# zhangmozhe/Deep-Exemplar-based-Video-Colorization

Hardware: AMD Instinct MI355X
Metric: colorized frames/sec/GPU at 216x384; correlation HBM GB/s vs roofline (higher is better)
Workload: dtype f32

## Files before the change

deep-exemplar-based-video-colorization_amd/csrc/norm_pool.hip:

```cpp
#include "common.h"
#include <algorithm>

thread_local char g_dvc_err[512] = {0};
char* dvc_err_buf() { return g_dvc_err; }

extern "C" int dvc_abi_version(void) { return DVC_ABI_VERSION; }
extern "C" const char* dvc_last_error(void) { return g_dvc_err; }

__device__ __forceinline__ double wave_sum_d(double v) {
#pragma unroll
    for (int off = 32; off > 0; off >>= 1) v += __shfl_xor(v, off, 64);
    return v;
}
__device__ __forceinline__ float wave_sum_f(float v) {
#pragma unroll
    for (int off = 32; off > 0; off >>= 1) v += __shfl_xor(v, off, 64);
    return v;
}

__device__ __forceinline__ double block_sum_d(double v, double* red) {
    v = wave_sum_d(v);
    int lane = threadIdx.x & 63, wave = threadIdx.x >> 6;
    __syncthreads();
    if (lane == 0) red[wave] = v;
    __syncthreads();
    double t = 0.0;
    int nw = blockDim.x >> 6;
    for (int i = 0; i < nw; ++i) t += red[i];
    return t;
}

__device__ __forceinline__ void plane_stats(const float* __restrict__ xp, int HW, float eps, float cs,
                                            double* red , float* sc_out, float* sh_out) {
    constexpr int VT = 1024;
    const int tid = threadIdx.x, nt = blockDim.x;
    const int nv = VT / nt;
    double s[4] = {0.0, 0.0, 0.0, 0.0}, q[4] = {0.0, 0.0, 0.0, 0.0};
    const int HW4 = ((reinterpret_cast<uintptr_t>(xp) & 15) == 0) ? (HW & ~3) : 0;
#pragma unroll
    for (int k = 0; k < 4; ++k) {
        if (k < nv) {
            const int v = tid + k * nt;
            int i = v * 4;
            for (; i + 3 * VT * 4 < HW4; i += 4 * VT * 4) {
                float4 x8[4];
#pragma unroll
                for (int u = 0; u < 4; ++u) x8[u] = *reinterpret_cast<const float4*>(xp + i + u * (VT * 4));
#pragma unroll
                for (int u = 0; u < 4; ++u) {
                    double a = x8[u].x, b = x8[u].y, cc = x8[u].z, d = x8[u].w;
                    s[k] += (a + b) + (cc + d);
                    q[k] += (a * a + b * b) + (cc * cc + d * d);
                }
            }
            for (; i < HW4; i += VT * 4) {
                float4 x4 = *reinterpret_cast<const float4*>(xp + i);
                double a = x4.x, b = x4.y, cc = x4.z, d = x4.w;
                s[k] += (a + b) + (cc + d);
                q[k] += (a * a + b * b) + (cc * cc + d * d);
            }
            for (int i = HW4 + v; i < HW; i += VT) {
                double a = xp[i];
                s[k] += a;
                q[k] += a * a;
            }
        }
    }
    const int lane = tid & 63, wave = tid >> 6, nw = nt >> 6;
#pragma unroll
    for (int k = 0; k < 4; ++k) {
        if (k < nv) {
            const double sk = wave_sum_d(s[k]), qk = wave_sum_d(q[k]);
            if (lane == 0) {
                red[wave + k * nw] = sk;
                red[16 + wave + k * nw] = qk;
            }
        }
    }
    __syncthreads();
    if (tid == 0) {
        double S = 0.0, Q = 0.0;
        for (int i = 0; i < VT / 64; ++i) {
            S += red[i];
            Q += red[16 + i];
        }
        const double mean = S / (double)HW;
        double var = Q / (double)HW - mean * mean;
        var = var < 0.0 ? 0.0 : var;
        const double rstd = 1.0 / sqrt(var + (double)eps);
        const double sc = rstd * (double)cs;
        red[32] = sc;
        red[33] = -mean * sc;
        red[34] = mean;
        red[35] = rstd;
    }
    __syncthreads();
    *sc_out = (float)red[32];
    *sh_out = (float)red[33];
}

__global__ __launch_bounds__(1024) void instnorm_stats_kernel(const float* __restrict__ x, int C, int HW,
                                                              long x_bs, float eps,
                                                              const float* __restrict__ chan_scale,
                                                              float* __restrict__ scale,
                                                              float* __restrict__ shift) {
    __shared__ double red[36];
    const int p = blockIdx.x;
    const int n = p / C, c = p - n * C;
    float sc, sh;
    plane_stats(x + (long)n * x_bs + (long)c * HW, HW, eps, chan_scale ? chan_scale[c] : 1.f, red, &sc, &sh);
    if (threadIdx.x == 0) {
        scale[p] = sc;
        shift[p] = sh;
    }
}

static int instnorm_block(int HW) { return HW >= 32768 ? 1024 : HW >= 8192 ? 512 : 256; }

extern "C" int dvc_instnorm_stats(const float* x, int32_t N, int32_t C, int32_t HW,
                                  int64_t x_batch_stride, float eps, const float* chan_scale,
                                  float* scale, float* shift, dvcStream stream) {
    DVC_REQUIRE(x && scale && shift && N > 0 && C > 0 && HW > 0, "dvc_instnorm_stats: bad argument");
    long bs = x_batch_stride ? x_batch_stride : (long)C * HW;
    hipLaunchKernelGGL(instnorm_stats_kernel, dim3(N * C), dim3(instnorm_block(HW)), 0, (hipStream_t)stream,
                       x, C, HW, bs, eps, chan_scale, scale, shift);
    DVC_CHECK_LAUNCH("dvc_instnorm_stats");
    return 0;
}

__device__ __forceinline__ void instnorm_apply_plane(const float* xp, const int p, const int n, const int c, double* red,
                                                     const float* __restrict__ res, const float* __restrict__ slope_ptr,
                                                     const float* __restrict__ chan_scale, float eps, int C, int H, int W,
                                                     int up, int sub, int rpad, long res_bs, long y_bs, float* __restrict__ y,
                                                     float* __restrict__ scale, float* __restrict__ shift,
                                                     const float* __restrict__ chan_scale2, int sub2, long y2_bs,
                                                     float* __restrict__ y2) {
    float sc, sh;
    plane_stats(xp, H * W, eps, chan_scale ? chan_scale[c] : 1.f, red, &sc, &sh);
    if (threadIdx.x == 0 && scale) {
        scale[p] = sc;
        shift[p] = sh;
    }
    if (y2) {
        const double sc2d = red[35] * (chan_scale2 ? (double)chan_scale2[c] : 1.0);
        const float sc2 = (float)sc2d, sh2 = (float)(-red[34] * sc2d);
        const int OH2 = sub2 == 2 ? (H + 1) / 2 : H, OW2 = sub2 == 2 ? (W + 1) / 2 : W;
        float* y2p = y2 + (long)n * y2_bs + (long)c * OH2 * OW2;
        for (int i = threadIdx.x; i < OH2 * OW2; i += blockDim.x) {
            const int oy = i / OW2, ox = i - oy * OW2;
            y2p[i] = xp[(oy * sub2) * W + ox * sub2] * sc2 + sh2;
        }
    }
    const bool has_act = slope_ptr != nullptr;
    const float slope = has_act ? *slope_ptr : 1.f;
    const float* rp = res ? res + (long)n * res_bs + (long)c * H * W : nullptr;
    const int VH = sub == 2 ? (H + 1) / 2 : H * up, VW = sub == 2 ? (W + 1) / 2 : W * up;
    const int OH = VH + 2 * rpad, OW = VW;
    float* yp = y + (long)n * y_bs + (long)c * OH * OW;
    const int total = OH * OW, nt = blockDim.x;
    if (up == 1 && sub == 1 && rpad == 0) {
        const bool v4 = ((reinterpret_cast<uintptr_t>(xp) | reinterpret_cast<uintptr_t>(yp) |
                          reinterpret_cast<uintptr_t>(rp)) & 15) == 0;
        const int T4 = v4 ? (total & ~3) : 0;
        auto piece = [&](const float4& v, const float4& r, int i) {
            float o[4] = {v.x * sc + sh, v.y * sc + sh, v.z * sc + sh, v.w * sc + sh};
            if (rp) { o[0] += r.x; o[1] += r.y; o[2] += r.z; o[3] += r.w; }
            if (has_act) {
#pragma unroll
                for (int k = 0; k < 4; ++k) o[k] = o[k] >= 0.f ? o[k] : o[k] * slope;
            }
            *reinterpret_cast<float4*>(yp + i) = make_float4(o[0], o[1], o[2], o[3]);
        };
        int i = threadIdx.x * 4;
        for (; i + nt * 4 < T4; i += 2 * nt * 4) {
            float4 v[2], r[2];
#pragma unroll
            for (int u = 0; u < 2; ++u) {
                v[u] = *reinterpret_cast<const float4*>(xp + i + u * nt * 4);
                r[u] = rp ? *reinterpret_cast<const float4*>(rp + i + u * nt * 4) : make_float4(0.f, 0.f, 0.f, 0.f);
            }
#pragma unroll
            for (int u = 0; u < 2; ++u) piece(v[u], r[u], i + u * nt * 4);
        }
        for (; i < T4; i += nt * 4) {
            const float4 v = *reinterpret_cast<const float4*>(xp + i);
            const float4 r = rp ? *reinterpret_cast<const float4*>(rp + i) : make_float4(0.f, 0.f, 0.f, 0.f);
            piece(v, r, i);
        }
        for (int i = T4 + threadIdx.x; i < total; i += nt) {
            float v = xp[i] * sc + sh;
            if (rp) v += rp[i];
            if (has_act) v = v >= 0.f ? v : v * slope;
            yp[i] = v;
        }
        return;
    }
    for (int i = threadIdx.x; i < total; i += nt) {
        int oy = i / OW, ox = i - oy * OW;
        int uy = oy - rpad;
        uy = uy < 0 ? 0 : (uy >= VH ? VH - 1 : uy);
        int sy = sub == 2 ? uy * 2 : (up == 1 ? uy : uy / up);
        int sx = sub == 2 ? ox * 2 : (up == 1 ? ox : ox / up);
        float v = xp[sy * W + sx] * sc + sh;
        if (rp) v += rp[sy * W + sx];
        if (has_act) v = v >= 0.f ? v : v * slope;
        yp[i] = v;
    }
}


__global__ __launch_bounds__(1024) void instnorm_apply_kernel(const float* __restrict__ x,
                                                              const float* __restrict__ res,
                                                              const float* __restrict__ slope_ptr,
                                                              const float* __restrict__ chan_scale, float eps,
                                                              int C, int H, int W, int up, int sub, int rpad,
                                                              long x_bs, long res_bs, long y_bs,
                                                              float* __restrict__ y, float* __restrict__ scale,
                                                              float* __restrict__ shift,
                                                              const float* __restrict__ chan_scale2, int sub2,
                                                              long y2_bs, float* __restrict__ y2) {
    __shared__ double red[36];
    const int p = blockIdx.x;
    const int n = p / C, c = p - n * C;
    instnorm_apply_plane(x + (long)n * x_bs + (long)c * H * W, p, n, c, red, res, slope_ptr, chan_scale, eps, C, H, W, up, sub,
                         rpad, res_bs, y_bs, y, scale, shift, chan_scale2, sub2, y2_bs, y2);
}

__global__ __launch_bounds__(1024) void instnorm_apply_partials_kernel(const float* __restrict__ part, int S, long slab,
                                                                       const float* __restrict__ bias, int act, float act_slope,
                                                                       const float* __restrict__ act_slope_ptr,
                                                                       const float* __restrict__ res,
                                                                       const float* __restrict__ slope_ptr,
                                                                       const float* __restrict__ chan_scale, float eps,
                                                                       int C, int H, int W, int up, int sub, int rpad,
                                                                       long res_bs, long y_bs,
                                                                       float* __restrict__ y, float* __restrict__ scale,
                                                                       float* __restrict__ shift,
                                                                       const float* __restrict__ chan_scale2, int sub2,
                                                                       long y2_bs, float* __restrict__ y2) {
    __shared__ double red[36];
// ... 28 lines not shown
    }
    __syncthreads();
    instnorm_apply_plane(plane, p, n, c, red, res, slope_ptr, chan_scale, eps, C, H, W, up, sub, rpad, res_bs, y_bs, y, scale,
                         shift, chan_scale2, sub2, y2_bs, y2);
}

extern "C" int dvc_instnorm_apply(const float* x, const float* residual, const float* slope_ptr,
                                  const float* chan_scale, float eps, int32_t N, int32_t C, int32_t H,
                                  int32_t W, int32_t up, int32_t sub, int32_t rpad, int64_t x_batch_stride,
                                  int64_t res_batch_stride, int64_t y_batch_stride, float* y,
                                  float* scale_out, float* shift_out, const float* chan_scale2, int32_t sub2,
                                  float* y2, dvcStream stream) {
    DVC_REQUIRE(x && y && N > 0 && C > 0 && H > 0 && W > 0, "dvc_instnorm_apply: bad argument");
    DVC_REQUIRE(!y2 || ((sub2 == 1 || sub2 == 2) && y2 != x && y2 != y), "dvc_instnorm_apply: bad second output");
    DVC_REQUIRE(!(y2 && x == y), "dvc_instnorm_apply: a second output excludes in-place operation");
    DVC_REQUIRE(up >= 1 && up <= 4 && (sub == 1 || sub == 2) && rpad >= 0 && !(up != 1 && sub != 1),
                "dvc_instnorm_apply: bad up/sub/rpad");
    DVC_REQUIRE(!(residual && (up != 1 || sub != 1)), "dvc_instnorm_apply: residual requires up == sub == 1");
    DVC_REQUIRE((scale_out == nullptr) == (shift_out == nullptr), "dvc_instnorm_apply: scale/shift come together");
    DVC_REQUIRE(!(x == y && (up != 1 || sub != 1 || rpad != 0)), "dvc_instnorm_apply: in place needs up == sub == 1, rpad == 0");
    const long VH = sub == 2 ? (H + 1) / 2 : (long)H * up, VW = sub == 2 ? (W + 1) / 2 : (long)W * up;
    const long OH = VH + 2 * rpad, OW = VW;
    long xbs = x_batch_stride ? x_batch_stride : (long)C * H * W;
    long rbs = res_batch_stride ? res_batch_stride : (long)C * H * W;
    long ybs = y_batch_stride ? y_batch_stride : (long)C * OH * OW;
    hipLaunchKernelGGL(instnorm_apply_kernel, dim3(N * C), dim3(instnorm_block(H * W)), 0, (hipStream_t)stream,
                       x, residual, slope_ptr, chan_scale, eps, C, H, W, up, sub, rpad, xbs, rbs, ybs, y,
                       scale_out, shift_out, chan_scale2, y2 ? sub2 : 1,
                       (long)C * (sub2 == 2 ? (H + 1) / 2 : H) * (sub2 == 2 ? (W + 1) / 2 : W), y2);
    DVC_CHECK_LAUNCH("dvc_instnorm_apply");
    return 0;
}

extern "C" int dvc_instnorm_apply_partials(const float* part, int32_t S, const float* bias, int32_t act, float act_slope,
                                           const float* act_slope_ptr, const float* residual, const float* slope_ptr,
                                           const float* chan_scale, float eps, int32_t N, int32_t C, int32_t H, int32_t W,
                                           int32_t up, int32_t sub, int32_t rpad, int64_t res_batch_stride,
                                           int64_t y_batch_stride, float* y, float* scale_out, float* shift_out,
                                           const float* chan_scale2, int32_t sub2, float* y2, dvcStream stream) {
    DVC_REQUIRE(part && y && S >= 1 && S <= 8 && N > 0 && C > 0 && H > 0 && W > 0, "dvc_instnorm_apply_partials: bad argument");
    DVC_REQUIRE((long)H * W <= 16384, "dvc_instnorm_apply_partials: plane of %d x %d does not fit the LDS image (<= 16384 elements)", H, W);
    DVC_REQUIRE(act == DVC_ACT_NONE || act == DVC_ACT_RELU || act == DVC_ACT_PRELU || act == DVC_ACT_LEAKY,
                "dvc_instnorm_apply_partials: unsupported activation %d", act);
    DVC_REQUIRE(!y2 || ((sub2 == 1 || sub2 == 2) && y2 != y), "dvc_instnorm_apply_partials: bad second output");
    DVC_REQUIRE(up >= 1 && up <= 4 && (sub == 1 || sub == 2) && rpad >= 0 && !(up != 1 && sub != 1),
                "dvc_instnorm_apply_partials: bad up/sub/rpad");
    DVC_REQUIRE(!(residual && (up != 1 || sub != 1)), "dvc_instnorm_apply_partials: residual requires up == sub == 1");
    DVC_REQUIRE((scale_out == nullptr) == (shift_out == nullptr), "dvc_instnorm_apply_partials: scale/shift come together");
    const long VH = sub == 2 ? (H + 1) / 2 : (long)H * up, VW = sub == 2 ? (W + 1) / 2 : (long)W * up;
    const long OH = VH + 2 * rpad, OW = VW;
    const long rbs = res_batch_stride ? res_batch_stride : (long)C * H * W;
    const long ybs = y_batch_stride ? y_batch_stride : (long)C * OH * OW;
    hipLaunchKernelGGL(instnorm_apply_partials_kernel, dim3(N * C), dim3(H * W >= 4096 ? 1024 : 512), (size_t)H * W * sizeof(float),
                       (hipStream_t)stream, part, S, (long)N * C * H * W, bias, act, act_slope, act_slope_ptr, residual, slope_ptr,
                       chan_scale, eps, C, H, W, up, sub, rpad, rbs, ybs, y, scale_out, shift_out, chan_scale2, y2 ? sub2 : 1,
                       (long)C * (sub2 == 2 ? (H + 1) / 2 : H) * (sub2 == 2 ? (W + 1) / 2 : W), y2);
    DVC_CHECK_LAUNCH("dvc_instnorm_apply_partials");
    return 0;
}

#define INSTNORM_GROUP_MAX 4
struct InstNormGroupArgs {
    DvcInstNormItem item[INSTNORM_GROUP_MAX];
    int start[INSTNORM_GROUP_MAX + 1];
    int n;
};
// ... 372 lines not shown
```

deep-exemplar-based-video-colorization_amd/dvc_amd/_lib.py:

```python
import ctypes
import os

_HERE = os.path.dirname(os.path.abspath(__file__))
DEBUG_BUILD = os.environ.get("DVC_DEBUG_LIB", "0") == "1"
LIB_PATH = os.path.join(_HERE, "libdvc_hip_debug.so" if DEBUG_BUILD else "libdvc_hip.so")
ABI_VERSION = 20

c_float_p = ctypes.c_void_p
c_i32 = ctypes.c_int32
c_i64 = ctypes.c_int64


class DvcConvDesc(ctypes.Structure):
    _fields_ = [
        ("N", c_i32), ("Cin", c_i32), ("H", c_i32), ("W", c_i32),
        ("Cout", c_i32), ("ksize", c_i32), ("stride", c_i32), ("dil", c_i32),
        ("pad", c_i32), ("pad_mode", c_i32), ("in_up", c_i32), ("in_sub", c_i32),
        ("act", c_i32), ("act_slope", ctypes.c_float), ("in_prelu", c_i32), ("cfg", c_i32), ("split_k", c_i32),
        ("x_batch_stride", c_i64), ("y_batch_stride", c_i64), ("res_batch_stride", c_i64),
        ("flags", c_i32), ("w_batch_stride", c_i64),
    ]


class DvcConvGroupItem(ctypes.Structure):
# ... 12 lines not shown
        ("N", c_i32), ("C", c_i32), ("H", c_i32), ("W", c_i32), ("up", c_i32), ("sub", c_i32), ("rpad", c_i32),
        ("x_batch_stride", c_i64), ("res_batch_stride", c_i64), ("y_batch_stride", c_i64), ("y", ctypes.c_void_p),
    ]


_VP = ctypes.c_void_p
SIGNATURES = {
    "dvc_abi_version": (ctypes.c_int, []),
    "dvc_last_error": (ctypes.c_char_p, []),
    "dvc_conv2d_out_hw": (ctypes.c_int, [ctypes.POINTER(DvcConvDesc), ctypes.POINTER(c_i32), ctypes.POINTER(c_i32)]),
    "dvc_conv2d": (ctypes.c_int, [ctypes.POINTER(DvcConvDesc), _VP, _VP, _VP, _VP, _VP, _VP, _VP, _VP, _VP, _VP,
                                  ctypes.c_size_t, _VP]),
    "dvc_winograd_weight_floats": (ctypes.c_size_t, [c_i32, c_i32]),
    "dvc_winograd_pack_weight": (ctypes.c_int, [_VP, c_i32, c_i32, _VP, _VP]),
    "dvc_conv2d_winograd_split": (ctypes.c_int, [ctypes.POINTER(DvcConvDesc), ctypes.c_size_t, ctypes.POINTER(c_i32),
                                                ctypes.POINTER(c_i32)]),
    "dvc_conv2d_winograd": (ctypes.c_int, [ctypes.POINTER(DvcConvDesc), _VP, _VP, _VP, _VP, _VP, _VP, _VP,
                                           ctypes.c_size_t, _VP]),
    "dvc_conv2d_winograd_pool": (ctypes.c_int, [ctypes.POINTER(DvcConvDesc), _VP, _VP, _VP, _VP, _VP, _VP, c_i64, _VP,
                                                ctypes.c_size_t, _VP]),
    "dvc_conv2d_winograd_dual": (ctypes.c_int, [ctypes.POINTER(DvcConvDesc), ctypes.POINTER(DvcConvDesc), _VP, _VP, _VP, _VP, _VP,
                                                _VP, _VP, ctypes.c_size_t, _VP]),
    "dvc_conv2d_ws_eligible": (ctypes.c_int, [ctypes.POINTER(DvcConvDesc)]),
    "dvc_conv2d_ws_pack_weight": (ctypes.c_int, [_VP, c_i32, c_i32, _VP, _VP]),
    "dvc_conv2d_ws": (ctypes.c_int, [ctypes.POINTER(DvcConvDesc), _VP, _VP, _VP, _VP, _VP, _VP]),
    "dvc_conv2d_winograd_group": (ctypes.c_int, [ctypes.POINTER(DvcConvGroupItem), c_i32, _VP]),
    "dvc_instnorm_apply_group": (ctypes.c_int, [ctypes.POINTER(DvcInstNormItem), c_i32, _VP]),
    "dvc_conv1x1_small": (ctypes.c_int, [_VP, _VP, _VP, c_i32, c_i32, c_i32, c_i32, c_i32, _VP, _VP]),
    "dvc_instnorm_stats": (ctypes.c_int, [_VP, c_i32, c_i32, c_i32, c_i64, ctypes.c_float, _VP, _VP, _VP, _VP]),
    "dvc_affine_act": (ctypes.c_int, [_VP, _VP, _VP, _VP, _VP, c_i32, c_i32, c_i32, c_i32, c_i32, c_i32,
                                      c_i64, c_i64, c_i64, _VP, _VP]),
    "dvc_instnorm_apply": (ctypes.c_int, [_VP, _VP, _VP, _VP, ctypes.c_float, c_i32, c_i32, c_i32, c_i32, c_i32,
                                          c_i32, c_i32, c_i64, c_i64, c_i64, _VP, _VP, _VP, _VP, c_i32, _VP, _VP]),
    "dvc_cx_prepare": (ctypes.c_int, [_VP, _VP, c_i32, c_i32, c_i32, c_i32, ctypes.c_float, _VP, _VP, _VP, _VP]),
    "dvc_cx_rows": (ctypes.c_int, [_VP, c_i32, c_i64, c_i64, c_i32, c_i32, ctypes.c_float, _VP, _VP, _VP, _VP, _VP, _VP]),
    "dvc_cx_colmax": (ctypes.c_int, [_VP, c_i32, c_i64, c_i64, _VP, _VP, c_i32, c_i32, c_i32, ctypes.c_float, _VP, _VP, _VP]),
    "dvc_cx_finish": (ctypes.c_int, [_VP, c_i32, c_i32, _VP, _VP, _VP]),
    "dvc_cx_rows_tq": (ctypes.c_int, [_VP, c_i32, c_i64, c_i64, c_i64, _VP, _VP, _VP, c_i32, c_i32, c_i32, ctypes.c_float, _VP, _VP,
                                      _VP]),
    "dvc_cx_ds": (ctypes.c_int, [_VP, c_i32, c_i64, c_i64, c_i64, _VP, _VP, _VP, _VP, _VP, _VP, _VP, _VP, _VP, ctypes.c_float, c_i32,
                                 c_i32, c_i32, c_i32, c_i32, ctypes.c_float, _VP, _VP, _VP]),
    "dvc_cx_normalize_bwd": (ctypes.c_int, [_VP, _VP, _VP, c_i32, c_i32, c_i32, ctypes.c_float, _VP, _VP]),
    "dvc_instnorm_apply_partials": (ctypes.c_int, [_VP, c_i32, _VP, c_i32, ctypes.c_float, _VP, _VP, _VP, _VP, ctypes.c_float,
                                                   c_i32, c_i32, c_i32, c_i32, c_i32, c_i32, c_i32, c_i64, c_i64, _VP, _VP, _VP,
                                                   _VP, c_i32, _VP, _VP]),
    "dvc_maxpool2x2": (ctypes.c_int, [_VP, c_i32, c_i32, c_i32, _VP, _VP]),
    "dvc_avgpool2x2": (ctypes.c_int, [_VP, c_i32, c_i32, c_i32, _VP, _VP]),
    "dvc_avgpool4x4": (ctypes.c_int, [_VP, c_i32, c_i32, c_i32, _VP, _VP]),
    "dvc_upsample_nearest": (ctypes.c_int, [_VP, c_i32, c_i32, c_i32, c_i32, _VP, _VP]),
    "dvc_channel_l2norm": (ctypes.c_int, [_VP, c_i32, c_i32, c_i32, ctypes.c_float, _VP, _VP]),
    "dvc_channel_l2norm_multi": (ctypes.c_int, [_VP, _VP, _VP, _VP, c_i32, c_i32, ctypes.c_float, _VP]),
    "dvc_gray2rgb": (ctypes.c_int, [_VP, c_i32, c_i32, c_i64, _VP, _VP]),
    "dvc_lab2rgb": (ctypes.c_int, [_VP, c_i32, c_i32, ctypes.c_float, _VP, _VP]),
    "dvc_pack_color_input": (ctypes.c_int, [_VP, c_i64, _VP, _VP, _VP, c_i64, _VP, c_i64, c_i32, c_i32, _VP, _VP]),
    "dvc_upsample_bilinear2x": (ctypes.c_int, [_VP, c_i32, c_i32, c_i32, ctypes.c_float, _VP, _VP]),
    "dvc_lum_guide_u8": (ctypes.c_int, [_VP, c_i64, _VP, _VP]),
    "dvc_fgs_workspace_bytes": (ctypes.c_size_t, [c_i32, c_i32, c_i32, c_i32, c_i32]),
    "dvc_fgs_filter": (ctypes.c_int, [_VP, _VP, c_i32, c_i32, c_i32, c_i32, ctypes.c_float, ctypes.c_float, c_i32,
                                      ctypes.c_float, _VP, _VP, ctypes.c_size_t, _VP]),
    "dvc_lab2rgb_u8": (ctypes.c_int, [_VP, _VP, c_i32, c_i32, _VP, _VP]),
    "dvc_rgb8_to_lab": (ctypes.c_int, [_VP, c_i32, c_i32, _VP, _VP]),
    "dvc_center_pad_workspace_bytes": (ctypes.c_size_t, [c_i32, c_i32]),
    "dvc_center_pad_is_fused": (ctypes.c_int, [c_i32, c_i32, c_i32, c_i32]),
    "dvc_center_pad": (ctypes.c_int, [_VP, c_i32, c_i32, c_i32, c_i32, _VP, _VP, ctypes.c_size_t, _VP]),
    "dvc_corr_prepare": (ctypes.c_int, [_VP, c_i32, c_i32, c_i32, ctypes.c_float, _VP, _VP, _VP]),
    "dvc_corr_workspace_bytes": (ctypes.c_size_t, [c_i32, c_i32]),
# ... 86 lines not shown
```

deep-exemplar-based-video-colorization_amd/dvc_amd/ops.py:

```python
import ctypes
import os as _os
import sys
from typing import NamedTuple

import torch

from . import _lib
from ._lib import DvcConvDesc, DvcConvGroupItem, DvcInstNormItem

ACT_NONE, ACT_RELU, ACT_PRELU, ACT_LEAKY, ACT_TANH128 = 0, 1, 2, 3, 4
PAD_ZERO, PAD_REFLECT = 0, 1
EPS64 = sys.float_info.epsilon


def _p(t):
    return None if t is None else ctypes.c_void_p(t.data_ptr())


def _pv(t):
    return None if t is None else t.data_ptr()


_raw_stream = getattr(torch._C, "_cuda_getCurrentRawStream", None)
_raw_device = getattr(torch._C, "_cuda_getDevice", None)
# ... 107 lines not shown
    _Switch("fold_merge", "set_fold_merge", "_fold_merge", "DVC_FOLD_MERGE", "1", _on_if_1, True),
    _Switch("batch_plan_enabled", None, "_batch_plan", None, "0", _on_if_1, True),
    _Switch("direct_layers", None, "DEFAULT_DIRECT_LAYERS", "DVC_DIRECT_LAYERS", None, _layer_names, True),
)


def _flag_functions(var, getter, setter):
    g = globals()

    def get():
        return g[var]

    def set_(flag=True):
        g[var] = bool(flag)
    get.__name__ = get.__qualname__ = getter
    set_.__name__ = set_.__qualname__ = setter
    return get, set_


for _sw in _SWITCHES:
    globals()[_sw.var] = _sw.parse(_os.environ.get(_sw.env, _sw.default) if _sw.env else _sw.default)
    if _sw.setter:
        globals()[_sw.getter], globals()[_sw.setter] = _flag_functions(_sw.var, _sw.getter, _sw.setter)
del _sw


def launch_epoch():
    g = globals()
    return tuple(g[sw.getter]() for sw in _SWITCHES if sw.launch)


def autotune_enabled():
    return _autotune


def set_autotune(flag=True):
    global _autotune
    _autotune = bool(flag)
    if _autotune:
        _load_tuned()


def conv_algo():
    return _conv_algo


def set_conv_algo(algo):
    global _conv_algo
    if algo not in ("auto", "speed", "direct", "winograd"):
        raise ValueError("conv algo must be 'auto', 'speed', 'direct' or 'winograd'")
    _conv_algo = algo


def exemplar_memo_enabled():
    return _exemplar_memo != "off"


def exemplar_memo_mode():
    return _exemplar_memo


def set_exemplar_memo(flag=True):
    global _exemplar_memo
    _exemplar_memo = "verify" if flag == "verify" else ("on" if flag else "off")


# ... 504 lines not shown
    _need_all(x=x, chan_scale=chan_scale)
    N, C, H, W = x.shape
    scale = torch.empty(N * C, device=x.device, dtype=torch.float32)
    shift = torch.empty(N * C, device=x.device, dtype=torch.float32)
    _lib.check(lib.dvc_instnorm_stats(_p(x), N, C, H * W, 0, float(eps), _p(chan_scale), _p(scale), _p(shift),
                                      _stream()), "dvc_instnorm_stats")
    return scale, shift


def affine_act(x, scale, shift, *, residual=None, slope_t=None, up=1, rpad=0, out=None, out_batch_stride=0):
    lib = _lib.load()
    _need_all(x=x, scale=scale, shift=shift, residual=residual, slope=slope_t)
    N, C, H, W = x.shape
    if out is None:
        out = torch.empty((N, C, H * up + 2 * rpad, W * up), device=x.device, dtype=torch.float32)
    _lib.check(lib.dvc_affine_act(_p(x), _p(scale), _p(shift), _p(residual), _p(slope_t), N, C, H, W, up, rpad,
                                  0, 0, out_batch_stride, _p(out), _stream()), "dvc_affine_act")
    return out


def _instnorm_prep(x, chan_scale, residual, slope_t, up, sub, rpad, out):
    part = x if isinstance(x, ConvPartials) else None
    if part is not None:
        part.check_live()
    _need_all(x=None if part is not None else x, chan_scale=chan_scale, residual=residual, slope=slope_t)
    N, C, H, W = part.shape if part is not None else x.shape
    dev = part.device if part is not None else x.device
    VH, VW = ((H + 1) // 2, (W + 1) // 2) if sub == 2 else (H * up, W * up)
    if out is None:
        out = torch.empty((N, C, VH + 2 * rpad, VW), device=dev, dtype=torch.float32)
    return part, N, C, H, W, dev, out


def instnorm_apply(x, *, eps=1e-5, chan_scale=None, residual=None, slope_t=None, up=1, sub=1, rpad=0, out=None,
                   out_batch_stride=0, second=None, scale_out=None):
    lib = _lib.load()
    assert not isinstance(out, ConvPartials)
    part, N, C, H, W, dev, out = _instnorm_prep(x, chan_scale, residual, slope_t, up, sub, rpad, out)
    cs2, sub2, y2 = None, 1, None
    if second is not None:
        cs2, sub2 = second
        _need(cs2, "chan_scale2")
        y2 = torch.empty((N, C, (H + 1) // 2, (W + 1) // 2) if sub2 == 2 else (N, C, H, W), device=dev,
                         dtype=torch.float32)
    if part is not None:
        assert scale_out is None, "scale_out: materialise the convolution's output first (defer_reduce=False)"
        _lib.check(lib.dvc_instnorm_apply_partials(ctypes.c_void_p(part.data_ptr()), part.S, _p(part.bias), part.act,
                                                   part.act_slope, _p(part.act_slope_t), _p(residual), _p(slope_t),
                                                   _p(chan_scale), float(eps), N, C, H, W, up, sub, rpad, 0, out_batch_stride,
                                                   _p(out), None, None, _p(cs2), sub2, _p(y2), _stream()),
                   "dvc_instnorm_apply_partials")
        return out if second is None else (out, y2)
    shift_out = None
    if scale_out is not None:
        _need(scale_out, "scale_out")
        assert scale_out.numel() == N * C, (scale_out.shape, N, C)
        shift_out = torch.empty_like(scale_out)
    _lib.check(lib.dvc_instnorm_apply(_p(x), _p(residual), _p(slope_t), _p(chan_scale), float(eps), N, C, H, W, up,
                                      sub, rpad, 0, 0, out_batch_stride, _p(out), _p(scale_out), _p(shift_out), _p(cs2), sub2,
                                      _p(y2), _stream()),
               "dvc_instnorm_apply")
    return out if second is None else (out, y2)


def instnorm_apply_group(items):
    n = len(items)
    if not (_group_heads and 2 <= n <= 4):
        return [instnorm_apply(it["x"], **{k: v for k, v in it.items() if k != "x"}) for it in items]
    lib = _lib.load()
    arr = (DvcInstNormItem * n)()
    outs = []
    for i, it in enumerate(items):
        x = it["x"]
        residual, slope_t, chan_scale = it.get("residual"), it.get("slope_t"), it.get("chan_scale")
        up, sub, rpad = it.get("up", 1), it.get("sub", 1), it.get("rpad", 0)
        part, N, C, H, W, _dev, out = _instnorm_prep(x, chan_scale, residual, slope_t, up, sub, rpad, it.get("out"))
        a = arr[i]
        a.x = part.data_ptr() if part is not None else x.data_ptr()
        a.S = part.S if part is not None else 0
        a.bias = _pv(part.bias) if part is not None else None
        a.act = part.act if part is not None else ACT_NONE
        a.act_slope = part.act_slope if part is not None else 0.0
        a.act_slope_ptr = _pv(part.act_slope_t) if part is not None else None
        a.residual, a.slope_ptr, a.chan_scale = _pv(residual), _pv(slope_t), _pv(chan_scale)
        a.eps = float(it.get("eps", 1e-5))
        a.N, a.C, a.H, a.W, a.up, a.sub, a.rpad = N, C, H, W, up, sub, rpad
        a.x_batch_stride, a.res_batch_stride, a.y_batch_stride = 0, 0, it.get("out_batch_stride", 0)
        a.y = out.data_ptr()
        outs.append(out)
    _lib.check(lib.dvc_instnorm_apply_group(arr, n, _stream()), "dvc_instnorm_apply_group")
    return outs


def _pool(fn_name, x, k):
    lib = _lib.load()
    _need(x, "x")
    N, C, H, W = x.shape
    y = torch.empty((N, C, H // k, W // k), device=x.device, dtype=torch.float32)
    _lib.check(getattr(lib, fn_name)(_p(x), N * C, H, W, _p(y), _stream()), fn_name)
    return y

# ... 475 lines not shown
```

include/dvc_hip.h:

```cpp
#ifndef DVC_HIP_H
#define DVC_HIP_H

#include <stddef.h>
#include <stdint.h>

#ifdef __cplusplus
extern "C" {
#endif

#pragma GCC visibility push(default)

typedef void* dvcStream;

#define DVC_ABI_VERSION 20

int dvc_abi_version(void);
const char* dvc_last_error(void);

enum { DVC_ACT_NONE = 0, DVC_ACT_RELU = 1, DVC_ACT_PRELU = 2, DVC_ACT_LEAKY = 3, DVC_ACT_TANH128 = 4 };
enum { DVC_PAD_ZERO = 0, DVC_PAD_REFLECT = 1 };

typedef struct DvcConvDesc {
    int32_t N, Cin, H, W;
    int32_t Cout;
// ... 52 lines not shown

typedef struct DvcConvGroupItem {
    DvcConvDesc d;
    const float* x;
    const float* u_packed;
    const float* bias;
    const float* act_slope_ptr;
    const float* residual;
    float* y;
    void* workspace;
    size_t workspace_bytes;
} DvcConvGroupItem;
int dvc_conv2d_winograd_group(const DvcConvGroupItem* items, int32_t n_items, dvcStream stream);

int dvc_conv1x1_small(const float* x, const float* w, const float* bias, int32_t N, int32_t Cin,
                      int32_t HW, int32_t Cout, int32_t act, float* y, dvcStream stream);

int dvc_instnorm_stats(const float* x, int32_t N, int32_t C, int32_t HW, int64_t x_batch_stride,
                       float eps, const float* chan_scale, float* scale, float* shift,
                       dvcStream stream);

int dvc_affine_act(const float* x, const float* scale, const float* shift, const float* residual,
                   const float* slope_ptr, int32_t N, int32_t C, int32_t H, int32_t W, int32_t up,
                   int32_t rpad, int64_t x_batch_stride, int64_t res_batch_stride,
                   int64_t y_batch_stride, float* y, dvcStream stream);

int dvc_instnorm_apply(const float* x, const float* residual , const float* slope_ptr ,
                       const float* chan_scale , float eps, int32_t N, int32_t C, int32_t H,
                       int32_t W, int32_t up, int32_t sub, int32_t rpad, int64_t x_batch_stride,
                       int64_t res_batch_stride, int64_t y_batch_stride, float* y,
                       float* scale_out, float* shift_out,
                       const float* chan_scale2 , int32_t sub2, float* y2 ,
                       dvcStream stream);
int dvc_instnorm_apply_partials(const float* part, int32_t S, const float* bias, int32_t act, float act_slope,
                                const float* act_slope_ptr, const float* residual, const float* slope_ptr,
                                const float* chan_scale, float eps, int32_t N, int32_t C, int32_t H, int32_t W, int32_t up,
                                int32_t sub, int32_t rpad, int64_t res_batch_stride, int64_t y_batch_stride, float* y,
                                float* scale_out, float* shift_out, const float* chan_scale2, int32_t sub2, float* y2,
                                dvcStream stream);

typedef struct DvcInstNormItem {
    const float* x;
    int32_t S;
    const float* bias;
    int32_t act;
    float act_slope;
    const float* act_slope_ptr;
    const float* residual;
    const float* slope_ptr;
    const float* chan_scale;
    float eps;
    int32_t N, C, H, W, up, sub, rpad;
    int64_t x_batch_stride, res_batch_stride, y_batch_stride;
    float* y;
} DvcInstNormItem;
int dvc_instnorm_apply_group(const DvcInstNormItem* items, int32_t n_items, dvcStream stream);

int dvc_maxpool2x2(const float* x, int32_t planes, int32_t H, int32_t W, float* y, dvcStream stream);
int dvc_avgpool2x2(const float* x, int32_t planes, int32_t H, int32_t W, float* y, dvcStream stream);
int dvc_avgpool4x4(const float* x, int32_t planes, int32_t H, int32_t W, float* y, dvcStream stream);
int dvc_upsample_nearest(const float* x, int32_t planes, int32_t H, int32_t W, int32_t f, float* y,
                         dvcStream stream);
int dvc_channel_l2norm(const float* x, int32_t N, int32_t C, int32_t HW, float eps, float* y,
                       dvcStream stream);
#define DVC_L2NORM_MAX_TENSORS 8
int dvc_channel_l2norm_multi(const float* const* x, float* const* y, const int32_t* C, const int32_t* HW,
// ... 121 lines not shown
```

Baseline: 432.1.

## Split instance norm across workgroups for large planes with few channels

Adds a two-kernel instance-norm path. A stats kernel spreads each plane's sum and sum-of-squares over up to 16 workgroups into a workspace, then an apply kernel reduces them and normalizes slabs of the plane across many workgroups. It is chosen automatically when there are few planes of large spatial size, to fill the GPU instead of using one block per plane. It costs an extra launch and a second read of the input.

Measured after the change: 432.5 (median of 2 runs). No clear change (+0.1%).

```diff
diff --git a/deep-exemplar-based-video-colorization_amd/csrc/norm_pool.hip b/deep-exemplar-based-video-colorization_amd/csrc/norm_pool.hip
--- a/deep-exemplar-based-video-colorization_amd/csrc/norm_pool.hip
+++ b/deep-exemplar-based-video-colorization_amd/csrc/norm_pool.hip
@@ -30,42 +30,62 @@
     return t;
 }
 
+__device__ __forceinline__ void vthread_sums(const float* __restrict__ xp, int HW, int HW4, int v, double& s, double& q) {
+    constexpr int VT = 1024;
+    int i = v * 4;
+    for (; i + 3 * VT * 4 < HW4; i += 4 * VT * 4) {
+        float4 x8[4];
+#pragma unroll
+        for (int u = 0; u < 4; ++u) x8[u] = *reinterpret_cast<const float4*>(xp + i + u * (VT * 4));
+#pragma unroll
+        for (int u = 0; u < 4; ++u) {
+            double a = x8[u].x, b = x8[u].y, cc = x8[u].z, d = x8[u].w;
+            s += (a + b) + (cc + d);
+            q += (a * a + b * b) + (cc * cc + d * d);
+        }
+    }
+    for (; i < HW4; i += VT * 4) {
+        float4 x4 = *reinterpret_cast<const float4*>(xp + i);
+        double a = x4.x, b = x4.y, cc = x4.z, d = x4.w;
+        s += (a + b) + (cc + d);
+        q += (a * a + b * b) + (cc * cc + d * d);
+    }
+    for (int i = HW4 + v; i < HW; i += VT) {
+        double a = xp[i];
+        s += a;
+        q += a * a;
+    }
+}
+__device__ __forceinline__ int plane_hw4(const float* xp, int HW) {
+    return ((reinterpret_cast<uintptr_t>(xp) & 15) == 0) ? (HW & ~3) : 0;
+}
+__device__ __forceinline__ void plane_stats_finish(double* red, int HW, float eps, float cs) {
+    double S = 0.0, Q = 0.0;
+    for (int i = 0; i < 16; ++i) {
+        S += red[i];
+        Q += red[16 + i];
+    }
+    const double mean = S / (double)HW;
+    double var = Q / (double)HW - mean * mean;
+    var = var < 0.0 ? 0.0 : var;
+    const double rstd = 1.0 / sqrt(var + (double)eps);
+    const double sc = rstd * (double)cs;
+    red[32] = sc;
+    red[33] = -mean * sc;
+    red[34] = mean;
+    red[35] = rstd;
+}
+
 __device__ __forceinline__ void plane_stats(const float* __restrict__ xp, int HW, float eps, float cs,
                                             double* red , float* sc_out, float* sh_out) {
     constexpr int VT = 1024;
     const int tid = threadIdx.x, nt = blockDim.x;
     const int nv = VT / nt;
     double s[4] = {0.0, 0.0, 0.0, 0.0}, q[4] = {0.0, 0.0, 0.0, 0.0};
-    const int HW4 = ((reinterpret_cast<uintptr_t>(xp) & 15) == 0) ? (HW & ~3) : 0;
-#pragma unroll
-    for (int k = 0; k < 4; ++k) {
-        if (k < nv) {
-            const int v = tid + k * nt;
-            int i = v * 4;
-            for (; i + 3 * VT * 4 < HW4; i += 4 * VT * 4) {
-                float4 x8[4];
-#pragma unroll
-                for (int u = 0; u < 4; ++u) x8[u] = *reinterpret_cast<const float4*>(xp + i + u * (VT * 4));
-#pragma unroll
-                for (int u = 0; u < 4; ++u) {
-                    double a = x8[u].x, b = x8[u].y, cc = x8[u].z, d = x8[u].w;
-                    s[k] += (a + b) + (cc + d);
-                    q[k] += (a * a + b * b) + (cc * cc + d * d);
-                }
-            }
-            for (; i < HW4; i += VT * 4) {
-                float4 x4 = *reinterpret_cast<const float4*>(xp + i);
-                double a = x4.x, b = x4.y, cc = x4.z, d = x4.w;
-                s[k] += (a + b) + (cc + d);
-                q[k] += (a * a + b * b) + (cc * cc + d * d);
-            }
-            for (int i = HW4 + v; i < HW; i += VT) {
-                double a = xp[i];
-                s[k] += a;
-                q[k] += a * a;
-            }
-        }
-    }
+    const int HW4 = plane_hw4(xp, HW);
+#pragma unroll
+    for (int k = 0; k < 4; ++k)
+        if (k < nv) vthread_sums(xp, HW, HW4, tid + k * nt, s[k], q[k]);
     const int lane = tid & 63, wave = tid >> 6, nw = nt >> 6;
 #pragma unroll
     for (int k = 0; k < 4; ++k) {
@@ -78,22 +98,7 @@
         }
     }
     __syncthreads();
-    if (tid == 0) {
-        double S = 0.0, Q = 0.0;
-        for (int i = 0; i < VT / 64; ++i) {
-            S += red[i];
-            Q += red[16 + i];
-        }
-        const double mean = S / (double)HW;
-        double var = Q / (double)HW - mean * mean;
-        var = var < 0.0 ? 0.0 : var;
-        const double rstd = 1.0 / sqrt(var + (double)eps);
-        const double sc = rstd * (double)cs;
-        red[32] = sc;
-        red[33] = -mean * sc;
-        red[34] = mean;
-        red[35] = rstd;
-    }
+    if (tid == 0) plane_stats_finish(red, HW, eps, cs);
     __syncthreads();
     *sc_out = (float)red[32];
     *sh_out = (float)red[33];
@@ -128,6 +133,92 @@
     return 0;
 }
 
+__device__ __forceinline__ void slab_range(int total, int b, int B, int* lo, int* hi) {
+    const int per = ((total + B - 1) / B + 3) & ~3;
+    const long l = (long)b * per;
+    *lo = l < total ? (int)l : total;
+    *hi = l + per < total ? (int)(l + per) : total;
+}
+
+__device__ __forceinline__ void instnorm_apply_slab(const float* xp, const int n, const int c, const double* red, const int b,
+                                                    const int B, const float* __restrict__ res,
+                                                    const float* __restrict__ slope_ptr, int H, int W, int up, int sub, int rpad,
+                                                    long res_bs, long y_bs, float* __restrict__ y,
+                                                    const float* __restrict__ chan_scale2, int sub2, long y2_bs,
+                                                    float* __restrict__ y2) {
+    const float sc = (float)red[32], sh = (float)red[33];
+    if (y2) {
+        const double sc2d = red[35] * (chan_scale2 ? (double)chan_scale2[c] : 1.0);
+        const float sc2 = (float)sc2d, sh2 = (float)(-red[34] * sc2d);
+        const int OH2 = sub2 == 2 ? (H + 1) / 2 : H, OW2 = sub2 == 2 ? (W + 1) / 2 : W;
+        float* y2p = y2 + (long)n * y2_bs + (long)c * OH2 * OW2;
+        int lo2, hi2;
+        slab_range(OH2 * OW2, b, B, &lo2, &hi2);
+        for (int i = lo2 + threadIdx.x; i < hi2; i += blockDim.x) {
+            const int oy = i / OW2, ox = i - oy * OW2;
+            y2p[i] = xp[(oy * sub2) * W + ox * sub2] * sc2 + sh2;
+        }
+    }
+    const bool has_act = slope_ptr != nullptr;
+    const float slope = has_act ? *slope_ptr : 1.f;
+    const float* rp = res ? res + (long)n * res_bs + (long)c * H * W : nullptr;
+    const int VH = sub == 2 ? (H + 1) / 2 : H * up, VW = sub == 2 ? (W + 1) / 2 : W * up;
+    const int OH = VH + 2 * rpad, OW = VW;
+    float* yp = y + (long)n * y_bs + (long)c * OH * OW;
+    const int total = OH * OW, nt = blockDim.x;
+    int lo, hi;
+    slab_range(total, b, B, &lo, &hi);
+    if (up == 1 && sub == 1 && rpad == 0) {
+        const bool v4 = ((reinterpret_cast<uintptr_t>(xp) | reinterpret_cast<uintptr_t>(yp) |
+                          reinterpret_cast<uintptr_t>(rp)) & 15) == 0;
+        const int T4 = v4 ? (total & ~3) : 0;
+        const int vhi = hi < T4 ? hi : T4;
+        auto piece = [&](const float4& v, const float4& r, int i) {
+            float o[4] = {v.x * sc + sh, v.y * sc + sh, v.z * sc + sh, v.w * sc + sh};
+            if (rp) { o[0] += r.x; o[1] += r.y; o[2] += r.z; o[3] += r.w; }
+            if (has_act) {
+#pragma unroll
+                for (int k = 0; k < 4; ++k) o[k] = o[k] >= 0.f ? o[k] : o[k] * slope;
+            }
+            *reinterpret_cast<float4*>(yp + i) = make_float4(o[0], o[1], o[2], o[3]);
+        };
+        int i = lo + threadIdx.x * 4;
+        for (; i + nt * 4 < vhi; i += 2 * nt * 4) {
+            float4 v[2], r[2];
+#pragma unroll
+            for (int u = 0; u < 2; ++u) {
+                v[u] = *reinterpret_cast<const float4*>(xp + i + u * nt * 4);
+                r[u] = rp ? *reinterpret_cast<const float4*>(rp + i + u * nt * 4) : make_float4(0.f, 0.f, 0.f, 0.f);
+            }
+#pragma unroll
+            for (int u = 0; u < 2; ++u) piece(v[u], r[u], i + u * nt * 4);
+        }
+        for (; i < vhi; i += nt * 4) {
+            const float4 v = *reinterpret_cast<const float4*>(xp + i);
+            const float4 r = rp ? *reinterpret_cast<const float4*>(rp + i) : make_float4(0.f, 0.f, 0.f, 0.f);
+            piece(v, r, i);
+        }
+        for (int i = (lo > T4 ? lo : T4) + threadIdx.x; i < hi; i += nt) {
+            float v = xp[i] * sc + sh;
+            if (rp) v += rp[i];
+            if (has_act) v = v >= 0.f ? v : v * slope;
+            yp[i] = v;
+        }
+        return;
+    }
+    for (int i = lo + threadIdx.x; i < hi; i += nt) {
+        int oy = i / OW, ox = i - oy * OW;
+        int uy = oy - rpad;
+        uy = uy < 0 ? 0 : (uy >= VH ? VH - 1 : uy);
+        int sy = sub == 2 ? uy * 2 : (up == 1 ? uy : uy / up);
+        int sx = sub == 2 ? ox * 2 : (up == 1 ? ox : ox / up);
+        float v = xp[sy * W + sx] * sc + sh;
+        if (rp) v += rp[sy * W + sx];
+        if (has_act) v = v >= 0.f ? v : v * slope;
+        yp[i] = v;
+    }
+}
+
 __device__ __forceinline__ void instnorm_apply_plane(const float* xp, const int p, const int n, const int c, double* red,
                                                      const float* __restrict__ res, const float* __restrict__ slope_ptr,
                                                      const float* __restrict__ chan_scale, float eps, int C, int H, int W,
@@ -141,71 +232,7 @@
         scale[p] = sc;
         shift[p] = sh;
     }
-    if (y2) {
-        const double sc2d = red[35] * (chan_scale2 ? (double)chan_scale2[c] : 1.0);
-        const float sc2 = (float)sc2d, sh2 = (float)(-red[34] * sc2d);
-        const int OH2 = sub2 == 2 ? (H + 1) / 2 : H, OW2 = sub2 == 2 ? (W + 1) / 2 : W;
-        float* y2p = y2 + (long)n * y2_bs + (long)c * OH2 * OW2;
-        for (int i = threadIdx.x; i < OH2 * OW2; i += blockDim.x) {
-            const int oy = i / OW2, ox = i - oy * OW2;
-            y2p[i] = xp[(oy * sub2) * W + ox * sub2] * sc2 + sh2;
-        }
-    }
-    const bool has_act = slope_ptr != nullptr;
-    const float slope = has_act ? *slope_ptr : 1.f;
-    const float* rp = res ? res + (long)n * res_bs + (long)c * H * W : nullptr;
-    const int VH = sub == 2 ? (H + 1) / 2 : H * up, VW = sub == 2 ? (W + 1) / 2 : W * up;
-    const int OH = VH + 2 * rpad, OW = VW;
-    float* yp = y + (long)n * y_bs + (long)c * OH * OW;
-    const int total = OH * OW, nt = blockDim.x;
-    if (up == 1 && sub == 1 && rpad == 0) {
-        const bool v4 = ((reinterpret_cast<uintptr_t>(xp) | reinterpret_cast<uintptr_t>(yp) |
-                          reinterpret_cast<uintptr_t>(rp)) & 15) == 0;
-        const int T4 = v4 ? (total & ~3) : 0;
-        auto piece = [&](const float4& v, const float4& r, int i) {
-            float o[4] = {v.x * sc + sh, v.y * sc + sh, v.z * sc + sh, v.w * sc + sh};
-            if (rp) { o[0] += r.x; o[1] += r.y; o[2] += r.z; o[3] += r.w; }
-            if (has_act) {
-#pragma unroll
-                for (int k = 0; k < 4; ++k) o[k] = o[k] >= 0.f ? o[k] : o[k] * slope;
-            }
-            *reinterpret_cast<float4*>(yp + i) = make_float4(o[0], o[1], o[2], o[3]);
-        };
-        int i = threadIdx.x * 4;
-        for (; i + nt * 4 < T4; i += 2 * nt * 4) {
-            float4 v[2], r[2];
-#pragma unroll
-            for (int u = 0; u < 2; ++u) {
-                v[u] = *reinterpret_cast<const float4*>(xp + i + u * nt * 4);
-                r[u] = rp ? *reinterpret_cast<const float4*>(rp + i + u * nt * 4) : make_float4(0.f, 0.f, 0.f, 0.f);
-            }
-#pragma unroll
-            for (int u = 0; u < 2; ++u) piece(v[u], r[u], i + u * nt * 4);
-        }
-        for (; i < T4; i += nt * 4) {
-            const float4 v = *reinterpret_cast<const float4*>(xp + i);
-            const float4 r = rp ? *reinterpret_cast<const float4*>(rp + i) : make_float4(0.f, 0.f, 0.f, 0.f);
-            piece(v, r, i);
-        }
-        for (int i = T4 + threadIdx.x; i < total; i += nt) {
-            float v = xp[i] * sc + sh;
-            if (rp) v += rp[i];
-            if (has_act) v = v >= 0.f ? v : v * slope;
-            yp[i] = v;
-        }
-        return;
-    }
-    for (int i = threadIdx.x; i < total; i += nt) {
-        int oy = i / OW, ox = i - oy * OW;
-        int uy = oy - rpad;
-        uy = uy < 0 ? 0 : (uy >= VH ? VH - 1 : uy);
-        int sy = sub == 2 ? uy * 2 : (up == 1 ? uy : uy / up);
-        int sx = sub == 2 ? ox * 2 : (up == 1 ? ox : ox / up);
-        float v = xp[sy * W + sx] * sc + sh;
-        if (rp) v += rp[sy * W + sx];
-        if (has_act) v = v >= 0.f ? v : v * slope;
-        yp[i] = v;
-    }
+    instnorm_apply_slab(xp, n, c, red, 0, 1, res, slope_ptr, H, W, up, sub, rpad, res_bs, y_bs, y, chan_scale2, sub2, y2_bs, y2);
 }
 
 
@@ -300,6 +327,110 @@
     return 0;
 }
 
+__global__ __launch_bounds__(512) void instnorm_split_stats_kernel(const float* __restrict__ x, int C, int HW, long x_bs, int G,
+                                                                   double* __restrict__ ws) {
+    const int p = blockIdx.x / G, j = blockIdx.x - p * G;
+    const int n = p / C, c = p - n * C;
+    const float* xp = x + (long)n * x_bs + (long)c * HW;
+    const int v = j * blockDim.x + threadIdx.x;
+    double s = 0.0, q = 0.0;
+    vthread_sums(xp, HW, plane_hw4(xp, HW), v, s, q);
+    s = wave_sum_d(s);
+    q = wave_sum_d(q);
+    if ((threadIdx.x & 63) == 0) *reinterpret_cast<double2*>(ws + ((long)p * 16 + (v >> 6)) * 2) = make_double2(s, q);
+}
+
+__global__ __launch_bounds__(256) void instnorm_split_apply_kernel(const float* __restrict__ x, const float* __restrict__ res,
+                                                                   const float* __restrict__ slope_ptr,
+                                                                   const float* __restrict__ chan_scale, float eps, int C, int H,
+                                                                   int W, int up, int sub, int rpad, long x_bs, long res_bs,
+                                                                   long y_bs, float* __restrict__ y, float* __restrict__ scale,
+                                                                   float* __restrict__ shift,
+                                                                   const float* __restrict__ chan_scale2, int sub2, long y2_bs,
+                                                                   float* __restrict__ y2, const double* __restrict__ ws, int B) {
+    __shared__ double red[36];
+    const int p = blockIdx.x / B, b = blockIdx.x - p * B;
+    const int n = p / C, c = p - n * C;
+    if (threadIdx.x < 32) red[(threadIdx.x & 1) * 16 + (threadIdx.x >> 1)] = ws[(long)p * 32 + threadIdx.x];
+    __syncthreads();
+    if (threadIdx.x == 0) {
+        plane_stats_finish(red, H * W, eps, chan_scale ? chan_scale[c] : 1.f);
+        if (scale && b == 0) {
+            scale[p] = (float)red[32];
+            shift[p] = (float)red[33];
+        }
+    }
+    __syncthreads();
+    instnorm_apply_slab(x + (long)n * x_bs + (long)c * H * W, n, c, red, b, B, res, slope_ptr, H, W, up, sub, rpad, res_bs, y_bs,
+                        y, chan_scale2, sub2, y2_bs, y2);
+}
+
+#define INSTNORM_SPLIT_MAX_PLANES 128
+#define INSTNORM_SPLIT_MIN_HW 82944
+#define INSTNORM_SPLIT_STATS_WGS 1024
+#define INSTNORM_SPLIT_APPLY_WGS 2048
+#define INSTNORM_SPLIT_SLAB_MIN 4096
+struct InstNormPlan { int G, B; };
+static InstNormPlan instnorm_plan(long planes, long HW, long outputs, int force_G) {
+    InstNormPlan pl = {1, 1};
+    if (force_G > 0) pl.G = force_G;
+    else if (planes <= INSTNORM_SPLIT_MAX_PLANES && HW >= INSTNORM_SPLIT_MIN_HW)
+        while (pl.G < 16 && planes * pl.G < INSTNORM_SPLIT_STATS_WGS) pl.G *= 2;
+    if (pl.G > 1) {
+        const long by_chip = (INSTNORM_SPLIT_APPLY_WGS + planes - 1) / planes, by_size = (outputs + INSTNORM_SPLIT_SLAB_MIN - 1) / INSTNORM_SPLIT_SLAB_MIN;
+        pl.B = (int)std::max(1L, std::min(std::min(by_chip, by_size), 64L));
+    }
+    return pl;
+}
+
+extern "C" int dvc_instnorm_split_plan(int64_t planes, int64_t HW) {
+    return planes > 0 && HW > 0 ? instnorm_plan(planes, HW, HW, 0).G : 1;
+}
+
+extern "C" int dvc_instnorm_apply_split(const float* x, const float* residual, const float* slope_ptr,
+                                        const float* chan_scale, float eps, int32_t N, int32_t C, int32_t H,
+                                        int32_t W, int32_t up, int32_t sub, int32_t rpad, int64_t x_batch_stride,
+                                        int64_t res_batch_stride, int64_t y_batch_stride, float* y,
+                                        float* scale_out, float* shift_out, const float* chan_scale2, int32_t sub2,
+                                        float* y2, int32_t split, void* workspace, size_t workspace_bytes, dvcStream stream) {
+    DVC_REQUIRE(split == 0 || split == 1 || split == 2 || split == 4 || split == 8 || split == 16,
+                "dvc_instnorm_apply_split: split %d is not 0 (planned), 1, 2, 4, 8 or 16", split);
+    DVC_REQUIRE(N > 0 && C > 0 && H > 0 && W > 0 && up >= 1 && up <= 4 && (sub == 1 || sub == 2) && rpad >= 0,
+                "dvc_instnorm_apply_split: bad argument");
+    const long planes = (long)N * C;
+    const long VH = sub == 2 ? (H + 1) / 2 : (long)H * up, VW = sub == 2 ? (W + 1) / 2 : (long)W * up;
+    const long OH = VH + 2 * rpad, OW = VW;
+    const long out2 = y2 ? (long)(sub2 == 2 ? (H + 1) / 2 : H) * (sub2 == 2 ? (W + 1) / 2 : W) : 0;
+    const InstNormPlan pl = instnorm_plan(planes, (long)H * W, std::max(OH * OW, out2), split);
+    if (pl.G == 1)
+        return dvc_instnorm_apply(x, residual, slope_ptr, chan_scale, eps, N, C, H, W, up, sub, rpad, x_batch_stride,
+                                  res_batch_stride, y_batch_stride, y, scale_out, shift_out, chan_scale2, sub2, y2, stream);
+    DVC_REQUIRE(x && y, "dvc_instnorm_apply_split: bad argument");
+    DVC_REQUIRE(!y2 || ((sub2 == 1 || sub2 == 2) && y2 != x && y2 != y), "dvc_instnorm_apply_split: bad second output");
+    DVC_REQUIRE(!(y2 && x == y), "dvc_instnorm_apply_split: a second output excludes in-place operation");
+    DVC_REQUIRE(!(up != 1 && sub != 1), "dvc_instnorm_apply_split: bad up/sub/rpad");
+    DVC_REQUIRE(!(residual && (up != 1 || sub != 1)), "dvc_instnorm_apply_split: residual requires up == sub == 1");
+    DVC_REQUIRE((scale_out == nullptr) == (shift_out == nullptr), "dvc_instnorm_apply_split: scale/shift come together");
+    DVC_REQUIRE(!(x == y && (up != 1 || sub != 1 || rpad != 0)), "dvc_instnorm_apply_split: in place needs up == sub == 1, rpad == 0");
+    DVC_REQUIRE(workspace && (reinterpret_cast<uintptr_t>(workspace) & 15) == 0 &&
+                workspace_bytes >= (size_t)planes * DVC_INSTNORM_SPLIT_WS_BYTES_PER_PLANE,
+                "dvc_instnorm_apply_split: workspace of %zu bytes, 16-byte aligned, needed (%zu given)",
+                (size_t)planes * DVC_INSTNORM_SPLIT_WS_BYTES_PER_PLANE, workspace_bytes);
+    DVC_REQUIRE(planes * std::max(pl.G, pl.B) < (1L << 31) && OH * OW < (1L << 31), "dvc_instnorm_apply_split: too large");
+    long xbs = x_batch_stride ? x_batch_stride : (long)C * H * W;
+    long rbs = res_batch_stride ? res_batch_stride : (long)C * H * W;
+    long ybs = y_batch_stride ? y_batch_stride : (long)C * OH * OW;
+    double* ws = static_cast<double*>(workspace);
+    hipLaunchKernelGGL(instnorm_split_stats_kernel, dim3((unsigned)(planes * pl.G)), dim3(1024 / pl.G), 0, (hipStream_t)stream,
+                       x, C, H * W, xbs, pl.G, ws);
+    DVC_CHECK_LAUNCH("dvc_instnorm_apply_split (statistics)");
+    hipLaunchKernelGGL(instnorm_split_apply_kernel, dim3((unsigned)(planes * pl.B)), dim3(256), 0, (hipStream_t)stream,
+                       x, residual, slope_ptr, chan_scale, eps, C, H, W, up, sub, rpad, xbs, rbs, ybs, y, scale_out, shift_out,
+                       chan_scale2, y2 ? sub2 : 1, (long)C * out2, y2, ws, pl.B);
+    DVC_CHECK_LAUNCH("dvc_instnorm_apply_split (apply)");
+    return 0;
+}
+
 extern "C" int dvc_instnorm_apply_partials(const float* part, int32_t S, const float* bias, int32_t act, float act_slope,
                                            const float* act_slope_ptr, const float* residual, const float* slope_ptr,
                                            const float* chan_scale, float eps, int32_t N, int32_t C, int32_t H, int32_t W,
diff --git a/deep-exemplar-based-video-colorization_amd/dvc_amd/_lib.py b/deep-exemplar-based-video-colorization_amd/dvc_amd/_lib.py
--- a/deep-exemplar-based-video-colorization_amd/dvc_amd/_lib.py
+++ b/deep-exemplar-based-video-colorization_amd/dvc_amd/_lib.py
@@ -68,6 +68,10 @@
                                       c_i64, c_i64, c_i64, _VP, _VP]),
     "dvc_instnorm_apply": (ctypes.c_int, [_VP, _VP, _VP, _VP, ctypes.c_float, c_i32, c_i32, c_i32, c_i32, c_i32,
                                           c_i32, c_i32, c_i64, c_i64, c_i64, _VP, _VP, _VP, _VP, c_i32, _VP, _VP]),
+    "dvc_instnorm_apply_split": (ctypes.c_int, [_VP, _VP, _VP, _VP, ctypes.c_float, c_i32, c_i32, c_i32, c_i32, c_i32,
+                                                c_i32, c_i32, c_i64, c_i64, c_i64, _VP, _VP, _VP, _VP, c_i32, _VP, c_i32, _VP,
+                                                ctypes.c_size_t, _VP]),
+    "dvc_instnorm_split_plan": (ctypes.c_int, [c_i64, c_i64]),
     "dvc_cx_prepare": (ctypes.c_int, [_VP, _VP, c_i32, c_i32, c_i32, c_i32, ctypes.c_float, _VP, _VP, _VP, _VP]),
     "dvc_cx_rows": (ctypes.c_int, [_VP, c_i32, c_i64, c_i64, c_i32, c_i32, ctypes.c_float, _VP, _VP, _VP, _VP, _VP, _VP]),
     "dvc_cx_colmax": (ctypes.c_int, [_VP, c_i32, c_i64, c_i64, _VP, _VP, c_i32, c_i32, c_i32, ctypes.c_float, _VP, _VP, _VP]),
diff --git a/deep-exemplar-based-video-colorization_amd/dvc_amd/ops.py b/deep-exemplar-based-video-colorization_amd/dvc_amd/ops.py
--- a/deep-exemplar-based-video-colorization_amd/dvc_amd/ops.py
+++ b/deep-exemplar-based-video-colorization_amd/dvc_amd/ops.py
@@ -163,6 +163,21 @@
 
 def autotune_enabled():
     return _autotune
+
+
+_instnorm_split = 0
+INSTNORM_SPLIT_WS_BYTES_PER_PLANE = 256
+
+
+def instnorm_split():
+    return _instnorm_split
+
+
+def set_instnorm_split(G=0):
+    global _instnorm_split
+    if G not in (0, 1, 2, 4, 8, 16):
+        raise ValueError(f"dvc_amd: instnorm split {G!r} is not one of 0, 1, 2, 4, 8, 16")
+    _instnorm_split = G
 
 
 def set_autotune(flag=True):
@@ -733,8 +748,20 @@
     return part, N, C, H, W, dev, out
 
 
+_instnorm_plans = {}
+
+
+def _instnorm_G(planes, HW):
+    if _instnorm_split:
+        return _instnorm_split
+    G = _instnorm_plans.get((planes, HW))
+    if G is None:
+        G = _instnorm_plans[(planes, HW)] = _lib.load().dvc_instnorm_split_plan(planes, HW)
+    return G
+
+
 def instnorm_apply(x, *, eps=1e-5, chan_scale=None, residual=None, slope_t=None, up=1, sub=1, rpad=0, out=None,
-                   out_batch_stride=0, second=None, scale_out=None):
+                   out_batch_stride=0, second=None, scale_out=None, split=None):
     lib = _lib.load()
     assert not isinstance(out, ConvPartials)
     part, N, C, H, W, dev, out = _instnorm_prep(x, chan_scale, residual, slope_t, up, sub, rpad, out)
@@ -757,6 +784,15 @@
         _need(scale_out, "scale_out")
         assert scale_out.numel() == N * C, (scale_out.shape, N, C)
         shift_out = torch.empty_like(scale_out)
+    G = _instnorm_G(N * C, H * W) if split is None else split
+    if G > 1:
+        nbytes = N * C * INSTNORM_SPLIT_WS_BYTES_PER_PLANE
+        ws = _workspace(dev, max(nbytes, 1 << 18), "instnorm")
+        _lib.check(lib.dvc_instnorm_apply_split(_p(x), _p(residual), _p(slope_t), _p(chan_scale), float(eps), N, C, H, W, up,
+                                                sub, rpad, 0, 0, out_batch_stride, _p(out), _p(scale_out), _p(shift_out),
+                                                _p(cs2), sub2, _p(y2), G, _p(ws), ws.numel(), _stream()),
+                   "dvc_instnorm_apply_split")
+        return out if second is None else (out, y2)
     _lib.check(lib.dvc_instnorm_apply(_p(x), _p(residual), _p(slope_t), _p(chan_scale), float(eps), N, C, H, W, up,
                                       sub, rpad, 0, 0, out_batch_stride, _p(out), _p(scale_out), _p(shift_out), _p(cs2), sub2,
                                       _p(y2), _stream()),
@@ -767,7 +803,7 @@
 def instnorm_apply_group(items):
     n = len(items)
     if not (_group_heads and 2 <= n <= 4):
-        return [instnorm_apply(it["x"], **{k: v for k, v in it.items() if k != "x"}) for it in items]
+        return [instnorm_apply(it["x"], split=1, **{k: v for k, v in it.items() if k != "x"}) for it in items]
     lib = _lib.load()
     arr = (DvcInstNormItem * n)()
     outs = []
diff --git a/include/dvc_hip.h b/include/dvc_hip.h
--- a/include/dvc_hip.h
+++ b/include/dvc_hip.h
@@ -108,6 +108,13 @@
                        float* scale_out, float* shift_out,
                        const float* chan_scale2 , int32_t sub2, float* y2 ,
                        dvcStream stream);
+#define DVC_INSTNORM_SPLIT_WS_BYTES_PER_PLANE 256
+int dvc_instnorm_apply_split(const float* x, const float* residual, const float* slope_ptr, const float* chan_scale, float eps,
+                             int32_t N, int32_t C, int32_t H, int32_t W, int32_t up, int32_t sub, int32_t rpad,
+                             int64_t x_batch_stride, int64_t res_batch_stride, int64_t y_batch_stride, float* y,
+                             float* scale_out, float* shift_out, const float* chan_scale2, int32_t sub2, float* y2,
+                             int32_t split, void* workspace, size_t workspace_bytes, dvcStream stream);
+int dvc_instnorm_split_plan(int64_t planes, int64_t HW);
 int dvc_instnorm_apply_partials(const float* part, int32_t S, const float* bias, int32_t act, float act_slope,
                                 const float* act_slope_ptr, const float* residual, const float* slope_ptr,
                                 const float* chan_scale, float eps, int32_t N, int32_t C, int32_t H, int32_t W, int32_t up,
```
